# tebartsch/numpy-quant

Measured on AMD Instinct MI355X. Metric: quantized-int8 samples/sec (ViT-tiny, batch 256) + MatMul GOPS vs int8-MFMA peak, higher is better.
Workload: dtype int8; 1 GPU; vit_image_classifier (reference models/vit graph, ViT-Base/16-224), QModel.__call__ (fused plan), int8, batch 256/GPU; model=vit_image_classifier_no_weights.onnx (ViT-Base/16-224), global_batch=256, seq_len=197, parallelism=replicas x1, executor=fused plan, hipGraph replay

## Files before the change

include/nqk.h:

```cpp
#ifndef NQK_H
#define NQK_H

#include <stddef.h>
#include <stdint.h>

#ifdef __cplusplus
extern "C" {
#endif

enum nqk_dtype { NQK_I8 = 1, NQK_I16 = 2, NQK_I32 = 3, NQK_I64 = 4, NQK_F32 = 5 };

enum nqk_zp_flags {
  NQK_ZP_NONE = 0,
  NQK_ZP_SCALAR = 1,
  NQK_ZP_ROW = 2,
  NQK_ZP_COL = 4,
  NQK_ZP_KCONST = 8,
  NQK_ZP_FULL = 16
};

int nqk_init(int device);
int nqk_device_count(int* count);
const char* nqk_last_error(void);
int nqk_malloc(void** ptr, size_t bytes);
// ... 145 lines not shown
  int64_t ln_zp;
} nqk_epilogue;
int nqk_pack_b(const int8_t* bt, int8_t* out, int64_t N, int64_t K, int64_t ldb);
int nqk_pack_b4(const int8_t* bt, uint8_t* out, int64_t N, int64_t K, int64_t ldb);
int nqk_pack_pg(const int8_t* bt, int8_t* out, int64_t N, int64_t K, int64_t ldb, int layout);
int nqk_pack_pg4(const int8_t* bt, uint8_t* out, int64_t N, int64_t K, int64_t ldb, int layout);
int nqk_gelu_lut_build(float s_out, int64_t zp_out, int32_t bit_width, float div, float add1, float mul2, void* lut,
                       float* k_out, int32_t* n_out);
int nqk_gelu_lut_capacity(void);
int nqk_gelu_lut_check(float s_out, int64_t zp_out, int32_t bit_width, float div, float add1, float mul2,
                       const void* lut, const float* k, int32_t n, uint64_t* mismatches);
int nqk_qgemm_fused(int epi, const int8_t* a, const int8_t* bt, int64_t batch, int64_t M, int64_t N, int64_t K,
                    int64_t lda, int64_t ldb, const int64_t* bmap, int64_t a_mat_stride, int64_t b_mat_stride,
                    const nqk_epilogue* params);
int nqk_qgemm_last_kernel(void);
int nqk_ln_quant(const float* x, const float* gamma, const float* beta, int8_t* out, int64_t rows, int64_t cols,
                 float eps, float scale, int64_t zp, int bit_width);
int nqk_softmax_quant(const float* x, int8_t* out, int64_t* rowsum, int64_t rows, int64_t cols, int64_t ldo,
                      float scale, int64_t zp, int bit_width);
int nqk_transpose_pad_i8(const int8_t* src, int8_t* dst, int64_t* rowsum, int64_t nb, int64_t R, int64_t C,
                         int64_t Rp);

typedef struct nqk_attention {
  int32_t heads, tokens, hdim, ld_out, bit_width, pad0;
  int64_t zq, zk;
  float s_qk, div;
  float s_p, s_pv;
  int64_t zp_p, zv;
  float s_ctx, pad1;
  int64_t zp_ctx;
} nqk_attention;
int nqk_attention_fused(const int8_t* q, const int8_t* k, const int8_t* v, int8_t* ctx, int64_t batch_heads,
                        const nqk_attention* params);

int nqk_selftest_fastmath(unsigned long long* counts_dev, uint32_t* examples_dev);
int nqk_selftest_gelu_filter(unsigned long long* stats_dev);

int nqk_comm_unique_id(void* id128);
int nqk_comm_init(const void* id128, int nranks, int rank);
int nqk_comm_bcast(void* buf, size_t bytes, int root);
int nqk_comm_gather(const void* send, void* recv, size_t bytes_per_rank, int root);
int nqk_comm_barrier(void);
int nqk_comm_destroy(void);

#ifdef __cplusplus
}
#endif
// ... 2 lines not shown
```

numpy-quant_amd/csrc/nqk_attn.hip:

```cpp
#include <type_traits>

#include "nqk_common.h"
#include "nqk_numerics.h"

#ifndef NQK_ATTN_DIAG
#define NQK_ATTN_DIAG 0
#endif
#ifndef NQK_ATTN_EXPW
#define NQK_ATTN_EXPW 4
#endif
#ifndef NQK_ATTN_PK
#define NQK_ATTN_PK 1
#endif
#ifndef NQK_ATTN_PQ2
#define NQK_ATTN_PQ2 1
#endif
#ifndef NQK_ATTN_EXP2
#define NQK_ATTN_EXP2 1
#endif
#ifndef NQK_ATTN_PREL
#define NQK_ATTN_PREL 1
#endif
#ifndef NQK_ATTN_PM_R
#define NQK_ATTN_PM_R 0x1.3p-22f
// ... 15 lines not shown
  (void)hipMemcpyFromSymbol(out, HIP_SYMBOL(g_attn_stats), 4 * sizeof(unsigned long long));
  const unsigned long long z[4] = {0, 0, 0, 0};
  if (reset) (void)hipMemcpyToSymbol(HIP_SYMBOL(g_attn_stats), z, sizeof(z));
  return 0;
}
#define NQK_ATTN_COUNT(i) \
  do { if ((threadIdx.x & 63) == 0) atomicAdd(&g_attn_stats[i], 1ull); } while (0)
#else
#define NQK_ATTN_COUNT(i) do { } while (0)
#endif
namespace {

typedef int v4i __attribute__((ext_vector_type(4)));
typedef int v16i __attribute__((ext_vector_type(16)));

struct AttnArgs {
  int T, H, ld_out, EST, PST, n2;
  int zq, zk, zp, zv;
  int kq, kp;
  float s_qk, div, s_p, s_pv, s_ctx;
  double rdiv, rs_p, zp_p, rs_ctx, zp_ctx, lo, hi;
  float inv_div, rs_ctx_f, zp_p_f, zp_ctx_f, lo_f, hi_f;
  float s_qkd;
};

__device__ __forceinline__ int swz64a(int row, int chunk) { return row * 64 + ((chunk ^ ((row >> 2) & 3)) << 4); }

__device__ __forceinline__ int sum16a(v4i c) {
  int s = __builtin_amdgcn_sdot4(c[0], 0x01010101, 0, false);
  s = __builtin_amdgcn_sdot4(c[1], 0x01010101, s, false);
  s = __builtin_amdgcn_sdot4(c[2], 0x01010101, s, false);
  return __builtin_amdgcn_sdot4(c[3], 0x01010101, s, false);
}

__device__ __forceinline__ float div_rc_w(float x, double rc) { return (float)((double)x * rc); }

__device__ __forceinline__ int quant_w(float x, float s, double rs, double zp, double lo, double hi) {
  const float t = div_rc_w(x, rs);
  const double u = zp + (double)t;
  return (int)__builtin_rint(__builtin_fmin(__builtin_fmax(u, lo), hi));
}

__device__ __forceinline__ int xor32i(int x) {
  const auto r = __builtin_amdgcn_permlane32_swap(x, x, false, false);
  return (threadIdx.x & 32) ? (int)r[0] : (int)r[1];
}
// ... 145 lines not shown
#pragma unroll
          for (int jj = 0; jj < 4; ++jj) qs[jj] = (int)o[jj];
        } else if constexpr (FAST) {
          v2f_t dd0, dd1;
          const v2f_t t0 = v2f_t{o[0], o[1]} * v2f_t{a.rs_ctx_f, a.rs_ctx_f};
          const v2f_t t1 = v2f_t{o[2], o[3]} * v2f_t{a.rs_ctx_f, a.rs_ctx_f};
          const v2f_t s0 = round_magic2(t0, a.lo_f - a.zp_ctx_f, a.hi_f - a.zp_ctx_f, 0x1.8p23f + a.zp_ctx_f, dd0);
          const v2f_t s1 = round_magic2(t1, a.lo_f - a.zp_ctx_f, a.hi_f - a.zp_ctx_f, 0x1.8p23f + a.zp_ctx_f, dd1);
          const float m0 = __builtin_fmaf(__builtin_fabsf(t0[0]), 0x1p-21f, __builtin_fabsf(dd0[0]));
          const float m1 = __builtin_fmaf(__builtin_fabsf(t0[1]), 0x1p-21f, __builtin_fabsf(dd0[1]));
          const float m2 = __builtin_fmaf(__builtin_fabsf(t1[0]), 0x1p-21f, __builtin_fabsf(dd1[0]));
          const float m3 = __builtin_fmaf(__builtin_fabsf(t1[1]), 0x1p-21f, __builtin_fabsf(dd1[1]));
          const uint32_t wm = __builtin_elementwise_max(__builtin_elementwise_max(__float_as_uint(m0), __float_as_uint(m1)),
                                                        __builtin_elementwise_max(__float_as_uint(m2), __float_as_uint(m3)));
          packed = pack4_low(s0, s1);
          if (__builtin_expect(__any(wm >= __float_as_uint(0x1.fffffcp-2f)), 0)) {
            NQK_ATTN_COUNT(3);
#pragma unroll
            for (int jj = 0; jj < 4; ++jj) {
              const int qv = quant_w(o[jj], a.s_ctx, a.rs_ctx, a.zp_ctx, a.lo, a.hi);
              packed = (packed & ~(0xffu << (8 * jj))) | ((uint32_t)(qv & 0xff) << (8 * jj));
            }
          }
          if (m < T) *reinterpret_cast<uint32_t*>(orow + d0) = packed;
          __builtin_amdgcn_sched_barrier(0);
          continue;
        } else {
#pragma unroll
          for (int jj = 0; jj < 4; ++jj) qs[jj] = quant_w(o[jj], a.s_ctx, a.rs_ctx, a.zp_ctx, a.lo, a.hi);
        }
#pragma unroll
        for (int jj = 0; jj < 4; ++jj) packed |= ((uint32_t)(qs[jj] & 0xff)) << (8 * jj);
        if (m < T) *reinterpret_cast<uint32_t*>(orow + d0) = packed;
        __builtin_amdgcn_sched_barrier(0);
      }
  };
  for (int rt = wave; rt < (TAILR ? NT - 1 : NT); rt += 4) {
    const int m0 = rt * 32, m = m0 + r32;
    v4i qb[2];
    const int nrowterm = q_rows(m, qb);
    int rp;
    v16i acc2[2];
    float e[NT][16];
    float mx = -__builtin_inff();
    float mn = __builtin_inff();
    int imx = INT32_MIN, imn = INT32_MAX;
#pragma unroll
    for (int c = 0; c < NT; ++c) {
      v16i acc;
#pragma unroll
      for (int qq = 0; qq < 4; ++qq) {
        if (pad_group(c, qq)) {
#pragma unroll
          for (int j = 0; j < 4; ++j) acc[4 * qq + j] = 0;
          continue;
        }
        const v4i ck = *reinterpret_cast<const v4i*>(colK + c * 32 + 8 * qq + 4 * h);
#pragma unroll
        for (int j = 0; j < 4; ++j) acc[4 * qq + j] = nrowterm - ck[j];
      }
// ... 341 lines not shown
          rp += qv;
          packed |= ((uint32_t)(qv & 0xff)) << (8 * j);
        }
        dw[qq] = (int)packed;
        __builtin_amdgcn_sched_barrier(0);
      }
      }
      const int xa = xor32i(h ? dw[0] : dw[2]);
      const int xb = xor32i(h ? dw[1] : dw[3]);
      v4i pb;
      if (h) { pb[0] = xa; pb[1] = dw[2]; pb[2] = xb; pb[3] = dw[3]; }
      else   { pb[0] = dw[0]; pb[1] = xa; pb[2] = dw[1]; pb[3] = xb; }
#pragma unroll
      for (int j = 0; j < 2; ++j) {
        const v4i va = *reinterpret_cast<const v4i*>(Vt + vt_row(j * 32 + r32) + (2 * c + h) * 16);
        if constexpr ((NQK_ATTN_DIAG & 32) != 0) acc2[j][c] ^= va[0] ^ pb[j];
        else acc2[j] = __builtin_amdgcn_mfma_i32_32x32x32_i8(va, pb, acc2[j], 0, 0, 0);
      }
    }
    rp += xor32i(rp);
    ctx_store(m, rp, acc2);
  }
  if constexpr (TAILR) {
    if (wave == (NT - 1) % 4) {
      const int rt = NT - 1, m = rt * 32 + r32;
      v4i qb[2];
      const int nrowterm = q_rows(m, qb);
      int rp;
      v16i acc2[2];
#pragma unroll
      for (int c = 0; c < NT; ++c) {
        v16i acc;
#pragma unroll
        for (int qq = 0; qq < 4; ++qq) {
          if (pad_group(c, qq)) {
#pragma unroll
            for (int j = 0; j < 4; ++j) acc[4 * qq + j] = 0;
            continue;
          }
          const v4i ck = *reinterpret_cast<const v4i*>(colK + c * 32 + 8 * qq + 4 * h);
#pragma unroll
          for (int j = 0; j < 4; ++j) acc[4 * qq + j] = nrowterm - ck[j];
        }
#pragma unroll
        for (int s = 0; s < 2; ++s) {
          const v4i ka = *reinterpret_cast<const v4i*>(Ks + swz64a(c * 32 + r32, 2 * s + h));
          acc = __builtin_amdgcn_mfma_i32_32x32x32_i8(ka, qb[s], acc, 0, 0, 0);
// ... 218 lines not shown
  if (tid < A16_KP) {
    const int8_t* kr = Ks + tid * 64;
    colK[tid] = (sum16a(*reinterpret_cast<const v4i*>(kr)) + sum16a(*reinterpret_cast<const v4i*>(kr + 16)) +
                 sum16a(*reinterpret_cast<const v4i*>(kr + 32)) + sum16a(*reinterpret_cast<const v4i*>(kr + 48))) * a.zq -
                a.kq;
  }
  if (tid < 256) {
    const int d = tid >> 2, ch = tid & 3;
    const int8_t* vr = Vt + (ch * 64 + d) * 64;
    int s = sum16a(*reinterpret_cast<const v4i*>(vr)) + sum16a(*reinterpret_cast<const v4i*>(vr + 16)) +
            sum16a(*reinterpret_cast<const v4i*>(vr + 32)) + sum16a(*reinterpret_cast<const v4i*>(vr + 48));
    s += __shfl_xor(s, 1, 64);
    s += __shfl_xor(s, 2, 64);
    if (ch == 0) colV[d] = s * a.zp - a.kp;
  }
  __syncthreads();

  const int fo = l15 * 64 + 16 * (g ^ a16_sw(l15));
  const float pqlo = a.lo_f - a.zp_p_f, pqhi = a.hi_f - a.zp_p_f, pmagic = 0x1.8p23f + a.zp_p_f;
  auto q_frag = [&](int rt) __attribute__((always_inline)) {
    const int mq = rt * 16 + l15;
    return *reinterpret_cast<const v4i*>(q + (mq < T ? mq : T - 1) * 64 + g * 16);
  };
  v4i qnext = q_frag(wave);
  for (int rt = wave; rt < NT; rt += NW) {
    const int m = rt * 16 + l15;
    const v4i qb = NQK_ATTN16_QPF ? qnext : q_frag(rt);
    int nrowterm;
    {
      int rq = sum16a(qb);
      rq += xor16i(rq);
      rq += xor32i(rq);
      nrowterm = -(rq * a.zk);
      asm volatile("" : "+v"(nrowterm));
    }
    float e[NT][4];
    int imx = INT32_MIN, imn = INT32_MAX;
    float mx = -__builtin_inff();
#pragma unroll
    for (int c = 0; c < NT; ++c) {
      const v4i ck = *reinterpret_cast<const v4i*>(colK + 16 * c + 4 * g);
      v4i acc = v4i{nrowterm - ck[0], nrowterm - ck[1], nrowterm - ck[2], nrowterm - ck[3]};
      const v4i ka = *reinterpret_cast<const v4i*>(Ks + c * 1024 + fo);
      acc = __builtin_amdgcn_mfma_i32_16x16x64_i8(ka, qb, acc, 0, 0, 0);
#pragma unroll
      for (int r = 0; r < 4; r += 2) {
        v2f_t y = v2f_t{(float)acc[r], (float)acc[r + 1]} * v2f_t{a.s_qkd, a.s_qkd};
        if (c == NT - 1) {
          const int n0 = 192 + 8 * (r >> 1) + 2 * g;
          y = y + v2f_t{n0 < T ? 0.0f : -__builtin_inff(), n0 + 1 < T ? 0.0f : -__builtin_inff()};
          mx = __builtin_fmaxf(mx, __builtin_fmaxf(y[0], y[1]));
        } else {
          imx = max(imx, max(acc[r], acc[r + 1]));
          imn = min(imn, min(acc[r], acc[r + 1]));
        }
        e[c][r] = y[0];
        e[c][r + 1] = y[1];
      }
    }
    if (NQK_ATTN16_QPF && rt + NW < NT) qnext = q_frag(rt + NW);
    mx = __builtin_fmaxf(mx, (float)imx * a.s_qkd);
    mx = __builtin_fmaxf(mx, xor16f(mx));
    mx = __builtin_fmaxf(mx, xor32f(mx));
    const float nm = -mx;
    const float mn = (float)imn * a.s_qkd;
    const bool esafe = __all(mn + nm >= NP_EXP_SAFE_LO);
#pragma unroll
    for (int c = 0; c < NT; ++c) {
#pragma unroll
      for (int r = 0; r < 4; r += 2) {
        const v2f_t xa = v2f_t{e[c][r], e[c][r + 1]} + v2f_t{nm, nm};
        const v2f_t x = (c < NT - 1 && esafe) ? np_expf_safe2(xa) : np_expf_nonpos2(xa);
        e[c][r] = x[0];
        e[c][r + 1] = x[1];
      }
      __builtin_amdgcn_sched_barrier(0);
    }
    float tot;
    {
      v2f_t a0 = v2f_t{e[0][0], e[0][1]}, a1 = v2f_t{e[6][0], e[6][1]};
      a0 = a0 + v2f_t{e[0][2], e[0][3]};
      a1 = a1 + v2f_t{e[6][2], e[6][3]};
#pragma unroll
// ... 103 lines not shown
      const v4i cv = *reinterpret_cast<const v4i*>(colV + d0);
      float o[4];
#pragma unroll
      for (int jj = 0; jj < 4; ++jj) o[jj] = (float)(acc2[mm][jj] - rowp - cv[jj]) * a.s_pv;
      v2f_t dd0, dd1;
      const v2f_t t0 = v2f_t{o[0], o[1]} * v2f_t{a.rs_ctx_f, a.rs_ctx_f};
      const v2f_t t1 = v2f_t{o[2], o[3]} * v2f_t{a.rs_ctx_f, a.rs_ctx_f};
      const v2f_t s0 = round_magic2(t0, a.lo_f - a.zp_ctx_f, a.hi_f - a.zp_ctx_f, 0x1.8p23f + a.zp_ctx_f, dd0);
      const v2f_t s1 = round_magic2(t1, a.lo_f - a.zp_ctx_f, a.hi_f - a.zp_ctx_f, 0x1.8p23f + a.zp_ctx_f, dd1);
      const float m0 = __builtin_fmaf(__builtin_fabsf(t0[0]), 0x1p-21f, __builtin_fabsf(dd0[0]));
      const float m1 = __builtin_fmaf(__builtin_fabsf(t0[1]), 0x1p-21f, __builtin_fabsf(dd0[1]));
      const float m2 = __builtin_fmaf(__builtin_fabsf(t1[0]), 0x1p-21f, __builtin_fabsf(dd1[0]));
      const float m3 = __builtin_fmaf(__builtin_fabsf(t1[1]), 0x1p-21f, __builtin_fabsf(dd1[1]));
      const uint32_t wm = __builtin_elementwise_max(__builtin_elementwise_max(__float_as_uint(m0), __float_as_uint(m1)),
                                                    __builtin_elementwise_max(__float_as_uint(m2), __float_as_uint(m3)));
      uint32_t packed = pack4_low(s0, s1);
      if (__builtin_expect(__any(wm >= __float_as_uint(0x1.fffffcp-2f)), 0)) {
#pragma unroll
        for (int jj = 0; jj < 4; ++jj) {
          const int qv = quant_w(o[jj], a.s_ctx, a.rs_ctx, a.zp_ctx, a.lo, a.hi);
          packed = (packed & ~(0xffu << (8 * jj))) | ((uint32_t)(qv & 0xff) << (8 * jj));
        }
      }
      if (m < T) *reinterpret_cast<uint32_t*>(orow + d0) = packed;
    }
  }
}
}
}

using namespace nqk;

extern "C" int nqk_attention_fused(const int8_t* q, const int8_t* k, const int8_t* v, int8_t* ctx,
                                   int64_t batch_heads, const nqk_attention* p) {
  if (batch_heads <= 0) return 0;
  const int T = p->tokens;
  if (p->hdim != 64) return fail("nqk_attention_fused: head dimension 64 expected");
  if (T < 1 || T > 224) return fail("nqk_attention_fused: 1 <= tokens <= 224 expected");
  if (p->heads < 1 || batch_heads % p->heads) return fail("nqk_attention_fused: batch_heads % heads != 0");
  if (p->ld_out < p->heads * 64) return fail("nqk_attention_fused: ld_out < heads * 64");
  if (p->bit_width < 2 || p->bit_width > 8) return fail("nqk_attention_fused: 2 <= bit_width <= 8 expected");
  auto small = [](int64_t z, int64_t lim) { return z >= -lim && z <= lim; };
  if (!small(p->zq, 4096) || !small(p->zk, 4096) || !small(p->zp_p, 1024) || !small(p->zv, 1024))
    return fail("nqk_attention_fused: zero points beyond the int32-exact range");
  if ((((uintptr_t)q) | ((uintptr_t)k) | ((uintptr_t)v)) & 15) return fail("nqk_attention_fused: unaligned Q/K/V");
  if ((((uintptr_t)ctx) & 3) || (p->ld_out & 3)) return fail("nqk_attention_fused: ctx / ld_out not 4-byte aligned");
  auto normal = [](float x) { return __builtin_fabsf(x) >= 0x1p-100f && __builtin_fabsf(x) <= 0x1p100f; };
  if (!normal(p->s_p) || !normal(p->s_ctx) || !normal(p->div))
    return fail("nqk_attention_fused: scales / divisor outside [2^-100, 2^100]");
  if (batch_heads > 0x7fffffff) return fail("nqk_attention_fused: too many (image, head) pairs");
  const int NT = (T + 31) / 32;
  AttnArgs a{};
  a.T = T;
  a.H = p->heads;
  a.ld_out = p->ld_out;
  int est = (T + 3) / 4 * 4;
  if (((est / 4) & 1) == 0) est += 4;
  a.EST = est;
  a.PST = NT * 32 + 16;
  a.n2 = 0;
  if (T > 128) {
    a.n2 = T / 2;
    a.n2 -= a.n2 % 8;
  }
  a.zq = (int)p->zq;
  a.zk = (int)p->zk;
  a.zp = (int)p->zp_p;
  a.zv = (int)p->zv;
  a.kq = a.zq * a.zk * 64;
  a.kp = a.zp * a.zv * T;
  a.s_qk = p->s_qk;
  a.div = p->div;
  a.rdiv = 1.0 / (double)p->div;
  a.s_p = p->s_p;
  a.rs_p = 1.0 / (double)p->s_p;
  a.zp_p = (double)p->zp_p;
// ... 50 lines not shown
```

numpy-quant_amd/numpy_quant/_lib.py:

```python
from __future__ import annotations

import ctypes
import os

_HERE = os.path.dirname(os.path.abspath(__file__))
LIB_PATH = os.path.join(_HERE, "libnqk.so")

NQK_I8, NQK_I16, NQK_I32, NQK_I64, NQK_F32 = 1, 2, 3, 4, 5
ZP_NONE, ZP_SCALAR, ZP_ROW, ZP_COL, ZP_KCONST, ZP_FULL = 0, 1, 2, 4, 8, 16
ADD, SUB, MUL, DIV = 0, 1, 2, 3
NEG, EXP, ERF, SQRT, RELU, SIGMOID, RECIP, TANH = range(8)
IMG_NHWC, IMG_NCHW = 0, 1

_p = ctypes.c_void_p
_i = ctypes.c_int
_l = ctypes.c_int64
_f = ctypes.c_float
_lp = ctypes.POINTER(ctypes.c_int64)

class Epilogue(ctypes.Structure):
    _fields_ = [("zp_flags", ctypes.c_int32), ("bit_width", ctypes.c_int32), ("group_cols", ctypes.c_int32),
                ("tokens", ctypes.c_int32), ("heads", ctypes.c_int32), ("hdim", ctypes.c_int32),
                ("ld_out", ctypes.c_int32), ("col_absmax", ctypes.c_int32),
                ("zpa", ctypes.c_int64), ("zpb", ctypes.c_int64), ("kdim", ctypes.c_int64),
                ("row", ctypes.c_void_p), ("col", ctypes.c_void_p),
                ("s_acc", ctypes.c_float * 3), ("s_out", ctypes.c_float * 3), ("zp_out", ctypes.c_int64 * 3),
                ("out", ctypes.c_void_p * 3), ("bias", ctypes.c_void_p), ("resid", ctypes.c_void_p),
                ("div", ctypes.c_float), ("add1", ctypes.c_float), ("mul2", ctypes.c_float),
                ("b_packed", ctypes.c_int32), ("colterm", ctypes.c_void_p), ("bt_pg", ctypes.c_void_p),
                ("gelu_lut", ctypes.c_void_p), ("lut_k", ctypes.c_float * 5), ("lut_n", ctypes.c_int32),
                ("col_l1max", ctypes.c_int32),
                ("ln_gamma", ctypes.c_void_p), ("ln_beta", ctypes.c_void_p), ("ln_out", ctypes.c_void_p),
                ("ln_eps", ctypes.c_float), ("ln_scale", ctypes.c_float), ("ln_zp", ctypes.c_int64)]


class Attention(ctypes.Structure):
    _fields_ = [("heads", ctypes.c_int32), ("tokens", ctypes.c_int32), ("hdim", ctypes.c_int32),
                ("ld_out", ctypes.c_int32), ("bit_width", ctypes.c_int32), ("pad0", ctypes.c_int32),
                ("zq", ctypes.c_int64), ("zk", ctypes.c_int64),
                ("s_qk", ctypes.c_float), ("div", ctypes.c_float), ("s_p", ctypes.c_float), ("s_pv", ctypes.c_float),
                ("zp_p", ctypes.c_int64), ("zv", ctypes.c_int64),
                ("s_ctx", ctypes.c_float), ("pad1", ctypes.c_float), ("zp_ctx", ctypes.c_int64)]


SIGNATURES = {
    "nqk_init": [_i],
    "nqk_device_count": [ctypes.POINTER(_i)],
    "nqk_malloc": [ctypes.POINTER(_p), ctypes.c_size_t],
    "nqk_free": [_p],
    "nqk_memcpy_h2d": [_p, _p, ctypes.c_size_t],
    "nqk_memcpy_d2h": [_p, _p, ctypes.c_size_t],
    "nqk_memcpy_d2d": [_p, _p, ctypes.c_size_t],
    "nqk_memset": [_p, _i, ctypes.c_size_t],
    "nqk_sync": [],
    "nqk_stream": [ctypes.POINTER(_p)],
    "nqk_set_stream": [_i],
    "nqk_stream_fork": [],
    "nqk_stream_join": [],
    "nqk_timer_start": [],
    "nqk_timer_stop": [],
    "nqk_timer_ms": [ctypes.POINTER(_f)],
# ... 135 lines not shown
```

numpy-quant_amd/numpy_quant/graph.py:

```python
from __future__ import annotations

import ctypes
from typing import List, Sequence, Union

import numpy as np

from . import _lib
from .device import POOL, DeviceArray, sync
from .tensor import FTensor


class DeviceGraph:

    def __init__(self, qmodel, example_inputs: Sequence[Union[np.ndarray, FTensor]], topk=None):
        _lib.ensure_init()
        from . import kernels as KM
        if KM.TIMER is not None:
            raise RuntimeError("DeviceGraph: kernels.TIMER is active; its events would be frozen into the graph")
        self.q = qmodel
        self.topk = topk
        self.staging: List[FTensor] = []
        for a in example_inputs:
            if isinstance(a, FTensor):
                self.staging.append(FTensor(a.dev.copy()))
            elif isinstance(a, np.ndarray) and a.dtype == np.float32:
                self.staging.append(FTensor(np.ascontiguousarray(a)))
            else:
                raise ValueError("DeviceGraph: float32 inputs only (int64 inputs are host tensors)")
        self.plan = None
        if qmodel._plan is not None or (qmodel.fuse and not qmodel.keep_values):
            from .plan import compile_plan
            self.plan = compile_plan(qmodel)
        self.exec = ctypes.c_void_p()
        self.outs: list = []
        self.blocks = []
        saved = qmodel._plan
        qmodel._plan = self.plan
        try:
            self._forward()
            sync()
            self.deq_cache = dict(qmodel._deq_cache)
            POOL.capture = []
            _lib.call("nqk_graph_begin")
            try:
                outs = self._forward()
            except BaseException:
                _lib.call("nqk_graph_abort")
                raise
            _lib.call("nqk_graph_end", ctypes.byref(self.exec))
            self.outs = outs
        finally:
            if POOL.capture is not None:
                self.blocks, POOL.capture = POOL.capture, None
            qmodel._plan = saved

# ... 46 lines not shown
```

numpy-quant_amd/numpy_quant/plan.py:

```python
from __future__ import annotations

import ctypes
import os
import math
from typing import Optional

import numpy as np

from . import _lib
from . import kernels as KM
from .device import DeviceArray
from .tensor import FTensor, QTensor

EPI_QKV, EPI_SCORES, EPI_PV, EPI_RESID, EPI_GELU = 0, 1, 2, 3, 4

_EPI_NAMES = {EPI_QKV: "qkv", EPI_SCORES: "scores", EPI_PV: "pv", EPI_RESID: "resid", EPI_GELU: "gelu"}

FUSED_ATTENTION = True
FUSED_EMBED = True
LN_GATHER = True
SPLIT_STREAMS = True


Epilogue = _lib.Epilogue
# ... 453 lines not shown
                                             4 * (n * hw * self.kk + self.kk * self.kout + n * (hw + 1) * self.kout)),
                         unit="flop32")
        m.add.outputs[0].data = FTensor(out)
        m.conv_out.data = FusedAway(m.conv_out.name)


class LnGather:

    def __init__(self, qmodel, ln):
        if ln.op != "LayerNormalization":
            raise NoMatch("LayerNormalization expected")
        out = ln.outputs[0]
        g = _only(out.outputs, "LN consumer")
        if g.op != "Gather" or g.inputs[0] is not out:
            raise NoMatch("Gather consumer expected")
        idx = g.inputs[1]
        if not (idx.inputs and idx.inputs[0].op == "Constant"):
            raise NoMatch("constant Gather indices expected")
        ax = int(ln.attrs.get("axis", -1))
        gax = int(g.attrs.get("axis", 0))
        if ax != -1 or gax in (-1,):
            raise NoMatch("LN over the last axis, Gather over another one")
        self.ln, self.g, self.nodes = ln, g, {ln, g}

    def run(self, qmodel, times=None, profile=False):
        from .model import onnx_operator_implementation
        x = self.ln.inputs[0].data
        if not isinstance(x, FTensor) or int(self.g.attrs.get("axis", 0)) % x.dev.ndim == x.dev.ndim - 1:
            raise ValueError("LN/Gather pushdown needs a float input gathered off the last axis")
        xs = x.take(self.g.inputs[1].data, axis=int(self.g.attrs.get("axis", 0)))
        args = [xs] + [qmodel._dequant_input(v) if isinstance(v.data, QTensor) else v.data for v in self.ln.inputs[1:]]
        self.g.outputs[0].data = onnx_operator_implementation("LayerNormalization", args, self.ln.attrs)[0]
        self.ln.outputs[0].data = FusedAway(self.ln.outputs[0].name)


class FusedLayer:
    def __init__(self, qmodel, m: LayerMatch):
        self.m = m
        self.bw = qmodel.bit_width
        qp = qmodel.quant_params
        deq = qmodel._dequant_input
        cf = lambda v: _const_float(qmodel, v)
        self.g1, self.be1 = cf(m.ln1.inputs[1]).dev, cf(m.ln1.inputs[2]).dev
        self.g2, self.be2 = cf(m.ln2.inputs[1]).dev, cf(m.ln2.inputs[2]).dev
        self.eps1 = _f32(m.ln1.attrs.get("epsilon", 1e-5))
        self.eps2 = _f32(m.ln2.attrs.get("epsilon", 1e-5))
        self.p_ln1, self.p_ln2 = qp[m.ln1_out.name], qp[m.ln2_out.name]
        self.p_sm, self.p_ctx, self.p_h = qp[m.sm_out.name], qp[m.rs3_out.name], qp[m.h_out.name]
        self.p_head = {r: qp[m.roles[r]["tr_out"].name] for r in "qkv"}
        bts, cols, biases, self.s_w = [], [], [], {}
        for r in "qkv":
            w = m.roles[r]["w"].data
            bt, col = w.weight_operand()
            bts.append(bt)
            cols.append(col)
            biases.append(deq(m.roles[r]["bias"]).dev)
# ... 10 lines not shown
        self.s_wo, self.s_w1, self.s_w2 = m.wo.data.scale, m.w1.data.scale, m.w2.data.scale
        self.bias_o, self.bias_1, self.bias_2 = deq(m.bo).dev, deq(m.b1).dev, deq(m.b2).dev
        self.F = self.bt_1.shape[0]
        self.bp = {k: _pack_b(b, self.bw) for k, b in (("qkv", self.bt_qkv), ("o", self.bt_o), ("1", self.bt_1),
                                                        ("2", self.bt_2))}
        self.bpg = {k: _pack_pg(b, self.bw, lay, nibbles=self.bp[k] is not None and self.bp[k][1] == 2)
                    for k, b, lay in (("qkv", self.bt_qkv, 0), ("o", self.bt_o, 1), ("1", self.bt_1, 0),
                                      ("2", self.bt_2, 1))}
        self.cmax = {k: _absmax(c) for k, c in (("qkv", self.col_qkv), ("o", self.col_o), ("1", self.col_1),
                                                 ("2", self.col_2))}
        self.l1max = {k: _l1max(b) for k, b in (("qkv", self.bt_qkv), ("o", self.bt_o), ("1", self.bt_1),
                                                 ("2", self.bt_2))}
        self.ct = {k: _colterm(c, _zp(p)) for k, c, p in (("qkv", self.col_qkv, self.p_ln1), ("o", self.col_o, self.p_ctx),
                                                          ("1", self.col_1, self.p_ln2), ("2", self.col_2, self.p_h))}
        if self.D != m.heads * m.hdim or self.bt_o.shape != (self.D, self.D) or self.bt_2.shape != (self.D, self.F):
            raise NoMatch("layer dimensions")
        self.glut = _gelu_lut(self.p_h, self.bw, m.gelu_div, m.gelu_add, m.gelu_mul)
        zs = [_zp(self.p_head["q"]), _zp(self.p_head["k"]), _zp(self.p_sm), _zp(self.p_head["v"])]
        self.attn_fused = (FUSED_ATTENTION and m.hdim == 64 and 1 <= m.tokens <= 224 and
                           abs(zs[0]) <= 4096 and abs(zs[1]) <= 4096 and abs(zs[2]) <= 1024 and abs(zs[3]) <= 1024)
        self.ln_fuse = self.D == 192 and not os.environ.get("NQK_NO_LNFUSE")
        self.next_ln = None
        self.ln1_by_prev = False

    def _epi(self, **kw) -> Epilogue:
        e = Epilogue()
        e.bit_width = self.bw
        e.group_cols = kw.pop("group_cols", 1 << 30)
        e.tokens, e.heads, e.hdim = self.m.tokens, self.m.heads, self.m.hdim
        e.div, e.add1, e.mul2 = kw.pop("div", 1.0), kw.pop("add1", 0.0), kw.pop("mul2", 1.0)
        for k, v in kw.items():
            if k in ("s_acc", "s_out", "zp_out", "out"):
                arr = getattr(e, k)
                for i, x in enumerate(v):
                    arr[i] = x
            else:
                setattr(e, k, v)
        return e

    @staticmethod
    def _ln_into(e, g, b, eps, p, out):
        e.ln_gamma, e.ln_beta, e.ln_out = g.ptr, b.ptr, out.ptr
        e.ln_eps, e.ln_scale, e.ln_zp = eps, _f32(p.scale), _zp(p)

    def _b(self, e, key, bt):
        bp = self.bp[key]
# ... 10 lines not shown
                      s_acc=[_f32(np.float32(pq.scale) * np.float32(pk.scale))], out=[w["s"].ptr], div=m.div)
        _gemm(EPI_SCORES, w["q"], w["k"], B * H, T, T, Dh, Dh, Dh, None, T * Dh, T * Dh, e)
        call("nqk_softmax_quant", w["s"].vp, w["p"].vp, None, B * H * T, T, Tp,
             _f32(self.p_sm.scale), _zp(self.p_sm), bw)
        e = self._epi(zp_flags=_lib.ZP_ROW | _lib.ZP_COL | _lib.ZP_KCONST, zpa=_zp(self.p_sm), zpb=_zp(pv_), kdim=T,
                      s_acc=[_f32(np.float32(self.p_sm.scale) * np.float32(pv_.scale))],
                      s_out=[_f32(self.p_ctx.scale)], zp_out=[_zp(self.p_ctx)], out=[w["ctx"].ptr], ld_out=D)
        _gemm(EPI_PV, w["p"], w["vt"], B * H, T, Dh, Tp, Tp, Tp, None, T * Tp, Dh * Tp, e)

    def run(self, ws: "Workspace", streams: Streams = _ONE_STREAM):
        m = self.m
        x = m.x_in.data
        if isinstance(x, QTensor):
            streams.join()
            x = x.dequantize()
        if not isinstance(x, FTensor):
            raise ValueError("fused layer input must be a float or quantized tensor")
        B, T, D = x.dev.shape
        if T != m.tokens or D != self.D:
            raise ValueError(f"layer input {x.dev.shape} does not match the graph ({m.tokens}, {self.D})")
        H, Dh, F = m.heads, m.hdim, self.F
        Tp = (T + 15) // 16 * 16
        w = ws.get(B, T, Tp, H, Dh, D, F, unfused_attention=not self.attn_fused)
        x2 = DeviceArray((B, T, D), np.float32)
        if not self.attn_fused:
            streams.join()
            streams = _ONE_STREAM
        streams.halves(B, lambda s_idx, i0, nb: self._run_part(w, x.dev, w["x1"], x2, i0, nb, s_idx, streams.parts))
        m.x_out.data = FTensor(x2)

    def _run_part(self, w, xd, x1d, x2d, i0, nb, s_idx=0, parts=1):
        m, bw = self.m, self.bw
        lag = _stream_lag() if parts > 1 else None
        if lag and s_idx > 0:
            _lib.call("nqk_event_wait", _lag_event(s_idx - 1))

        def mark(point):
            if lag == point and s_idx + 1 < parts:
                _lib.call("nqk_event_record", _lag_event(s_idx))
        T, D = m.tokens, self.D
        H, Dh, F = m.heads, m.hdim, self.F
        Mrows = nb * T
        Tp = (T + 15) // 16 * 16
        r0 = i0 * T

        def rows(arr, ncol):
            return arr.offset_view(r0 * ncol, (Mrows, ncol))

        x, x1, x2 = (rows(t.reshape((t.size // D, D)), D) for t in (xd, x1d, x2d))
        lnq, ln2q, ctx, hh = rows(w["lnq"], D), rows(w["ln2q"], D), rows(w["ctx"], D), rows(w["h"], F)
        hq = i0 * H * T * Dh
        q, k, v = (w[r].offset_view(hq, (nb * H * T, Dh)) for r in "qkv")
        call = _lib.call
        if not self.ln1_by_prev:
            _ln_quant(x, self.g1, self.be1, lnq, Mrows, D, self.eps1, self.p_ln1, bw)
        mark("ln1")
        s_a = np.float32(self.p_ln1.scale)
        e = self._epi(zp_flags=_lib.ZP_COL, zpa=_zp(self.p_ln1), group_cols=D, col=self.col_qkv.ptr,
                      col_absmax=self.cmax["qkv"], col_l1max=self.l1max["qkv"], colterm=_ptr(self.ct["qkv"]),
                      s_acc=[_f32(s_a * np.float32(self.s_w[r])) for r in "qkv"],
                      s_out=[_f32(self.p_head[r].scale) for r in "qkv"],
                      zp_out=[_zp(self.p_head[r]) for r in "qkv"],
                      out=[q.ptr, k.ptr, v.ptr], bias=self.bias_qkv.ptr)
        _gemm(EPI_QKV, lnq, self._b(e, "qkv", self.bt_qkv), 1, Mrows, 3 * D, D, D, D, None, 0, 0, e)
        mark("qkv")
        pq, pk, pv_ = self.p_head["q"], self.p_head["k"], self.p_head["v"]
        if self.attn_fused:
            a = _lib.Attention()
            a.heads, a.tokens, a.hdim, a.ld_out, a.bit_width = H, T, Dh, D, bw
            a.zq, a.zk = _zp(pq), _zp(pk)
            a.s_qk, a.div = _f32(np.float32(pq.scale) * np.float32(pk.scale)), m.div
            a.s_p, a.zp_p = _f32(self.p_sm.scale), _zp(self.p_sm)
            a.s_pv, a.zv = _f32(np.float32(self.p_sm.scale) * np.float32(pv_.scale)), _zp(pv_)
            a.s_ctx, a.zp_ctx = _f32(self.p_ctx.scale), _zp(self.p_ctx)
            t0 = KM.TIMER.begin() if KM.TIMER is not None else None
            call("nqk_attention_fused", q.vp, k.vp, v.vp, ctx.vp, nb * H, ctypes.byref(a))
            if t0 is not None:
                KM.TIMER.end("attention", t0, (2 * 2 * nb * H * T * T * Dh, 3 * nb * H * T * Dh + nb * T * D))
        else:
            self._attention_unfused(w, nb, T, Tp, H, Dh, D)
        mark("attn")
        e = self._epi(zp_flags=_lib.ZP_COL, zpa=_zp(self.p_ctx), col=self.col_o.ptr, col_absmax=self.cmax["o"], col_l1max=self.l1max["o"],
                      colterm=_ptr(self.ct["o"]),
                      s_acc=[_f32(np.float32(self.p_ctx.scale) * np.float32(self.s_wo))], bias=self.bias_o.ptr,
                      resid=x.ptr, out=[x1.ptr])
        if self.ln_fuse:
            self._ln_into(e, self.g2, self.be2, self.eps2, self.p_ln2, ln2q)
        _gemm(EPI_RESID, ctx, self._b(e, "o", self.bt_o), 1, Mrows, D, D, D, D, None, 0, 0, e)
        if not self.ln_fuse:
            _ln_quant(x1, self.g2, self.be2, ln2q, Mrows, D, self.eps2, self.p_ln2, bw)
        e = self._epi(zp_flags=_lib.ZP_COL, zpa=_zp(self.p_ln2), col=self.col_1.ptr, col_absmax=self.cmax["1"], col_l1max=self.l1max["1"],
                      colterm=_ptr(self.ct["1"]),
                      s_acc=[_f32(np.float32(self.p_ln2.scale) * np.float32(self.s_w1))], bias=self.bias_1.ptr,
                      s_out=[_f32(self.p_h.scale)], zp_out=[_zp(self.p_h)], out=[hh.ptr],
                      div=m.gelu_div, add1=m.gelu_add, mul2=m.gelu_mul)
        if self.glut is not None:
            e.gelu_lut, e.lut_n = self.glut[0].ptr, self.glut[2]
            for j, kv in enumerate(self.glut[1]):
                e.lut_k[j] = kv
        _gemm(EPI_GELU, ln2q, self._b(e, "1", self.bt_1), 1, Mrows, F, D, D, D, None, 0, 0, e)
        e = self._epi(zp_flags=_lib.ZP_COL, zpa=_zp(self.p_h), col=self.col_2.ptr, col_absmax=self.cmax["2"], col_l1max=self.l1max["2"],
                      colterm=_ptr(self.ct["2"]),
                      s_acc=[_f32(np.float32(self.p_h.scale) * np.float32(self.s_w2))], bias=self.bias_2.ptr,
                      resid=x1.ptr, out=[x2.ptr])
        nl = self.next_ln
        if nl is not None:
            self._ln_into(e, nl.g1, nl.be1, nl.eps1, nl.p_ln1, lnq)
        _gemm(EPI_RESID, hh, self._b(e, "2", self.bt_2), 1, Mrows, D, F, F, F, None, 0, 0, e)


def _pack_b(bt, bit_width=8):
    N, K = bt.shape
# ... 80 lines not shown
        raise ValueError("fused GEMM operands must be 16-byte padded")
    need_a = (batch - 1) * a_ms + (M - 1) * lda + K if batch > 1 else (M - 1) * lda + K
    need_b = (batch - 1) * b_ms + (N - 1) * ldb + K if batch > 1 else (N - 1) * ldb + K
    if e.b_packed:
        need_b = ((N + 255) // 256 * 256) * K // (2 if e.b_packed == 2 else 1)
    if need_a > a.size or need_b > bt.size * bt.dtype.itemsize:
        raise ValueError("fused GEMM operand smaller than its shape")
    t0 = KM.TIMER.begin() if KM.TIMER is not None else None
    _lib.call("nqk_qgemm_fused", epi, a.vp, bt.vp, batch, M, N, K, lda, ldb,
              _lib.i64arr(bmap) if bmap is not None else None, a_ms, b_ms, ctypes.byref(e))
    if t0 is not None:
        name = _EPI_NAMES[epi]
        out_b = 8 * M * N if epi == EPI_RESID else (M * N if epi in (EPI_QKV, EPI_GELU) else 0)
        if epi == EPI_RESID:
            name = "down" if K > N else "out"
        KM.TIMER.end("qgemm_" + name, t0, (2 * batch * M * N * K, batch * (M * K + N * K + out_b)))


class Workspace:

    def __init__(self):
        self.key = None
        self.bufs = {}

    def get(self, B, T, Tp, H, Dh, D, F, unfused_attention=True):
        key = (B, T, Tp, H, Dh, D, F)
        if key != self.key:
            M = B * T
            self.bufs = {
                "lnq": DeviceArray((M, D), np.int8), "ln2q": DeviceArray((M, D), np.int8),
                "q": DeviceArray((B * H * T, Dh), np.int8), "k": DeviceArray((B * H * T, Dh), np.int8),
                "v": DeviceArray((B * H * T, Dh), np.int8),
                "ctx": DeviceArray((M, D), np.int8), "h": DeviceArray((M, F), np.int8),
                "x1": DeviceArray((B, T, D), np.float32),
            }
            self.key = key
        if unfused_attention and "s" not in self.bufs:
            self.bufs.update({"vt": DeviceArray((B * H, Dh, Tp), np.int8),
                              "s": DeviceArray((B * H, T, T), np.float32),
                              "p": DeviceArray((B * H, T, Tp), np.int8)})
        return self.bufs


class FusedAwayError(RuntimeError):
    """Reading a FusedAway value."""


class FusedAway:

    def __init__(self, name):
        self.name = name

    def _error(self):
        return FusedAwayError(f"value {self.name!r} was computed inside a fused plan step and not kept; "
                              "set QModel.keep_values = True to read intermediates")

    def __getattr__(self, attr):
        if attr.startswith("__") and attr.endswith("__"):
            raise AttributeError(attr)
        raise self._error()

    def __array__(self, *args, **kwargs):
        raise self._error()

# ... 46 lines not shown
                    claimed[n] = layer
        placed = set()
        for node in qmodel.nodes:
            layer = claimed.get(node)
            if layer is None:
                self.steps.append(("node", node))
            elif isinstance(layer, LnGather):
                if node is layer.g:
                    self.steps.append(("ln_gather", layer))
            elif isinstance(layer, FusedEmbed):
                if node is layer.m.conv:
                    self.steps.append(("embed_pre", layer))
                elif node is layer.m.add:
                    self.steps.append(("embed", layer))
            elif id(layer) not in placed:
                placed.add(id(layer))
                self.steps.append(("layer", layer))
                self.fused += 1
        for (k0, a), (k1, b) in zip(self.steps, self.steps[1:]):
            if (k0 == "layer" and k1 == "layer" and a.ln_fuse and b.ln_fuse and b.m.x_in is a.m.x_out and
                    (a.D, a.F, a.m.heads, a.m.hdim, a.m.tokens, a.attn_fused) ==
                    (b.D, b.F, b.m.heads, b.m.hdim, b.m.tokens, b.attn_fused)):
                a.next_ln, b.ln1_by_prev = b, True
        self.internal = [v for node in qmodel.nodes if node in claimed for v in node.outputs]

    def run(self, qmodel, times=None, profile=False):
        streams = Streams(self.split, int(os.environ.get("NQK_STREAMS", "2")))
        for v in self.internal:
            v.data = FusedAway(v.name)
        try:
            for kind, obj in self.steps:
                if kind == "node":
                    streams.join()
                    qmodel._run_node(obj, times, profile)
                elif kind == "embed_pre":
                    obj.pre(qmodel)
                elif kind == "embed":
                    obj.run(qmodel, streams)
                elif kind == "ln_gather":
                    streams.join()
                    obj.run(qmodel, times, profile)
                else:
                    obj.run(self.ws, streams)
        finally:
            _lib.call("nqk_set_stream", 0)
            streams.join()


def compile_plan(qmodel) -> Plan:
    return Plan(qmodel)
```

Baseline: 29570 samples/s.

## Compute only CLS token rows in final transformer layer before LN/Gather

When the last layer's output only feeds a LayerNorm+Gather of token 0, the final layer now runs attention for just the first query row (new q_rows parameter in the fused attention kernel) and runs the out-projection/MLP on B rows instead of B*T. The full output becomes a lazily computed deferred tensor, or is fused away inside the graph executor. This removes the attention queries, out-proj and MLP work for the remaining tokens in the last layer. In exchange it adds CLS-specific workspace buffers, strided copies, and a plan rewrite that depends on the graph gathering index 0.

```diff
diff --git a/include/nqk.h b/include/nqk.h
--- a/include/nqk.h
+++ b/include/nqk.h
@@ -191,7 +191,7 @@
                          int64_t Rp);
 
 typedef struct nqk_attention {
-  int32_t heads, tokens, hdim, ld_out, bit_width, pad0;
+  int32_t heads, tokens, hdim, ld_out, bit_width, q_rows;
   int64_t zq, zk;
   float s_qk, div;
   float s_p, s_pv;
diff --git a/numpy-quant_amd/csrc/nqk_attn.hip b/numpy-quant_amd/csrc/nqk_attn.hip
--- a/numpy-quant_amd/csrc/nqk_attn.hip
+++ b/numpy-quant_amd/csrc/nqk_attn.hip
@@ -61,6 +61,7 @@
   double rdiv, rs_p, zp_p, rs_ctx, zp_ctx, lo, hi;
   float inv_div, rs_ctx_f, zp_p_f, zp_ctx_f, lo_f, hi_f;
   float s_qkd;
+  int QR;
 };
 
 __device__ __forceinline__ int swz64a(int row, int chunk) { return row * 64 + ((chunk ^ ((row >> 2) & 3)) << 4); }
@@ -252,7 +253,7 @@
               packed = (packed & ~(0xffu << (8 * jj))) | ((uint32_t)(qv & 0xff) << (8 * jj));
             }
           }
-          if (m < T) *reinterpret_cast<uint32_t*>(orow + d0) = packed;
+          if (m < a.QR) *reinterpret_cast<uint32_t*>(orow + d0) = packed;
           __builtin_amdgcn_sched_barrier(0);
           continue;
         } else {
@@ -261,11 +262,12 @@
         }
 #pragma unroll
         for (int jj = 0; jj < 4; ++jj) packed |= ((uint32_t)(qs[jj] & 0xff)) << (8 * jj);
-        if (m < T) *reinterpret_cast<uint32_t*>(orow + d0) = packed;
+        if (m < a.QR) *reinterpret_cast<uint32_t*>(orow + d0) = packed;
         __builtin_amdgcn_sched_barrier(0);
       }
   };
-  for (int rt = wave; rt < (TAILR ? NT - 1 : NT); rt += 4) {
+  const int ntq = (a.QR + 31) >> 5;
+  for (int rt = wave; rt < (TAILR ? min(ntq, NT - 1) : ntq); rt += 4) {
     const int m0 = rt * 32, m = m0 + r32;
     v4i qb[2];
     const int nrowterm = q_rows(m, qb);
@@ -653,7 +655,7 @@
     ctx_store(m, rp, acc2);
   }
   if constexpr (TAILR) {
-    if (wave == (NT - 1) % 4) {
+    if (wave == (NT - 1) % 4 && ntq == NT) {
       const int rt = NT - 1, m = rt * 32 + r32;
       v4i qb[2];
       const int nrowterm = q_rows(m, qb);
@@ -918,8 +920,9 @@
     const int mq = rt * 16 + l15;
     return *reinterpret_cast<const v4i*>(q + (mq < T ? mq : T - 1) * 64 + g * 16);
   };
+  const int ntq = (a.QR + 15) >> 4;
   v4i qnext = q_frag(wave);
-  for (int rt = wave; rt < NT; rt += NW) {
+  for (int rt = wave; rt < ntq; rt += NW) {
     const int m = rt * 16 + l15;
     const v4i qb = NQK_ATTN16_QPF ? qnext : q_frag(rt);
     int nrowterm;
@@ -954,7 +957,7 @@
         e[c][r + 1] = y[1];
       }
     }
-    if (NQK_ATTN16_QPF && rt + NW < NT) qnext = q_frag(rt + NW);
+    if (NQK_ATTN16_QPF && rt + NW < ntq) qnext = q_frag(rt + NW);
     mx = __builtin_fmaxf(mx, (float)imx * a.s_qkd);
     mx = __builtin_fmaxf(mx, xor16f(mx));
     mx = __builtin_fmaxf(mx, xor32f(mx));
@@ -1104,7 +1107,7 @@
           packed = (packed & ~(0xffu << (8 * jj))) | ((uint32_t)(qv & 0xff) << (8 * jj));
         }
       }
-      if (m < T) *reinterpret_cast<uint32_t*>(orow + d0) = packed;
+      if (m < a.QR) *reinterpret_cast<uint32_t*>(orow + d0) = packed;
     }
   }
 }
@@ -1119,6 +1122,7 @@
   const int T = p->tokens;
   if (p->hdim != 64) return fail("nqk_attention_fused: head dimension 64 expected");
   if (T < 1 || T > 224) return fail("nqk_attention_fused: 1 <= tokens <= 224 expected");
+  if (p->q_rows < 0 || p->q_rows > T) return fail("nqk_attention_fused: 0 <= q_rows <= tokens expected");
   if (p->heads < 1 || batch_heads % p->heads) return fail("nqk_attention_fused: batch_heads % heads != 0");
   if (p->ld_out < p->heads * 64) return fail("nqk_attention_fused: ld_out < heads * 64");
   if (p->bit_width < 2 || p->bit_width > 8) return fail("nqk_attention_fused: 2 <= bit_width <= 8 expected");
@@ -1134,6 +1138,7 @@
   const int NT = (T + 31) / 32;
   AttnArgs a{};
   a.T = T;
+  a.QR = p->q_rows ? p->q_rows : T;
   a.H = p->heads;
   a.ld_out = p->ld_out;
   int est = (T + 3) / 4 * 4;
diff --git a/numpy-quant_amd/numpy_quant/_lib.py b/numpy-quant_amd/numpy_quant/_lib.py
--- a/numpy-quant_amd/numpy_quant/_lib.py
+++ b/numpy-quant_amd/numpy_quant/_lib.py
@@ -36,7 +36,7 @@
 
 class Attention(ctypes.Structure):
     _fields_ = [("heads", ctypes.c_int32), ("tokens", ctypes.c_int32), ("hdim", ctypes.c_int32),
-                ("ld_out", ctypes.c_int32), ("bit_width", ctypes.c_int32), ("pad0", ctypes.c_int32),
+                ("ld_out", ctypes.c_int32), ("bit_width", ctypes.c_int32), ("q_rows", ctypes.c_int32),
                 ("zq", ctypes.c_int64), ("zk", ctypes.c_int64),
                 ("s_qk", ctypes.c_float), ("div", ctypes.c_float), ("s_p", ctypes.c_float), ("s_pv", ctypes.c_float),
                 ("zp_p", ctypes.c_int64), ("zv", ctypes.c_int64),
diff --git a/numpy-quant_amd/numpy_quant/graph.py b/numpy-quant_amd/numpy_quant/graph.py
--- a/numpy-quant_amd/numpy_quant/graph.py
+++ b/numpy-quant_amd/numpy_quant/graph.py
@@ -31,6 +31,9 @@
         if qmodel._plan is not None or (qmodel.fuse and not qmodel.keep_values):
             from .plan import compile_plan
             self.plan = compile_plan(qmodel)
+            for kind, step in self.plan.steps:
+                if kind == "layer":
+                    step.keep_deferred = False
         self.exec = ctypes.c_void_p()
         self.outs: list = []
         self.blocks = []
diff --git a/numpy-quant_amd/numpy_quant/plan.py b/numpy-quant_amd/numpy_quant/plan.py
--- a/numpy-quant_amd/numpy_quant/plan.py
+++ b/numpy-quant_amd/numpy_quant/plan.py
@@ -499,16 +499,54 @@
         if ax != -1 or gax in (-1,):
             raise NoMatch("LN over the last axis, Gather over another one")
         self.ln, self.g, self.nodes = ln, g, {ln, g}
+        self.cls_layer = None
+
+    def gathers_token0(self) -> bool:
+        idx = np.asarray(_const_node_value(self.g.inputs[1])[0])
+        return int(self.g.attrs.get("axis", 0)) == 1 and idx.size == 1 and int(idx.reshape(-1)[0]) == 0
 
     def run(self, qmodel, times=None, profile=False):
         from .model import onnx_operator_implementation
+        if self.cls_layer is not None:
+            c = self.cls_layer.cls_out.dev
+            idx = np.asarray(self.g.inputs[1].data.data)
+            xs = FTensor(c.reshape((c.shape[0],) + idx.shape + (c.shape[2],)))
+        else:
+            xs = self._gather()
+        args = [xs] + [qmodel._dequant_input(v) if isinstance(v.data, QTensor) else v.data for v in self.ln.inputs[1:]]
+        self.g.outputs[0].data = onnx_operator_implementation("LayerNormalization", args, self.ln.attrs)[0]
+        self.ln.outputs[0].data = FusedAway(self.ln.outputs[0].name)
+
+    def _gather(self):
         x = self.ln.inputs[0].data
         if not isinstance(x, FTensor) or int(self.g.attrs.get("axis", 0)) % x.dev.ndim == x.dev.ndim - 1:
             raise ValueError("LN/Gather pushdown needs a float input gathered off the last axis")
-        xs = x.take(self.g.inputs[1].data, axis=int(self.g.attrs.get("axis", 0)))
-        args = [xs] + [qmodel._dequant_input(v) if isinstance(v.data, QTensor) else v.data for v in self.ln.inputs[1:]]
-        self.g.outputs[0].data = onnx_operator_implementation("LayerNormalization", args, self.ln.attrs)[0]
-        self.ln.outputs[0].data = FusedAway(self.ln.outputs[0].name)
+        return x.take(self.g.inputs[1].data, axis=int(self.g.attrs.get("axis", 0)))
+
+
+class DeferredRows(FTensor):
+
+    def __init__(self, name, shape, thunk):
+        self.name, self._shape, self._thunk = name, tuple(shape), thunk
+        self._dev = self._host = None
+
+    @property
+    def dev(self):
+        if self._dev is None:
+            if self._thunk is None:
+                raise FusedAwayError(f"value {self.name!r}: only its token-0 rows were computed, and a later run "
+                                     "has reused the layer's workspace; read it before the next run, or set "
+                                     "QModel.keep_values = True")
+            self._dev, self._thunk = self._thunk(), None
+        return self._dev
+
+    @property
+    def shape(self):
+        from .tensor import ITensor
+        return ITensor(np.array(self._shape, dtype=np.int64))
+
+    def expire(self):
+        self._thunk = None
 
 
 class FusedLayer:
@@ -565,6 +603,10 @@
         self.ln_fuse = self.D == 192 and not os.environ.get("NQK_NO_LNFUSE")
         self.next_ln = None
         self.ln1_by_prev = False
+        self.cls_tail = False
+        self.keep_deferred = True
+        self.cls_out = None
+        self.deferred = None
 
     def _epi(self, **kw) -> Epilogue:
         e = Epilogue()
@@ -621,6 +663,9 @@
         H, Dh, F = m.heads, m.hdim, self.F
         Tp = (T + 15) // 16 * 16
         w = ws.get(B, T, Tp, H, Dh, D, F, unfused_attention=not self.attn_fused)
+        if self.cls_tail:
+            self._run_cls(ws, w, x, B, streams)
+            return
         x2 = DeviceArray((B, T, D), np.float32)
         if not self.attn_fused:
             streams.join()
@@ -628,7 +673,39 @@
         streams.halves(B, lambda s_idx, i0, nb: self._run_part(w, x.dev, w["x1"], x2, i0, nb, s_idx, streams.parts))
         m.x_out.data = FTensor(x2)
 
-    def _run_part(self, w, xd, x1d, x2d, i0, nb, s_idx=0, parts=1):
+    def _run_cls(self, ws, w, x, B, streams):
+        from .device import copy_strided
+        m = self.m
+        T, D = m.tokens, self.D
+        c = ws.cls(B, D, self.F)
+        out = DeviceArray((B, 1, D), np.float32)
+
+        def part(s_idx, i0, nb):
+            def rows(arr):
+                ncol = arr.shape[-1]
+                return arr.offset_view(i0 * ncol, (nb, ncol))
+            self._run_part(w, x.dev, None, None, i0, nb, s_idx, streams.parts, q_rows=1)
+            copy_strided(w["ctx"], c["ctx"], (nb, D), (T * D, 1), (D, 1), i0 * T * D, i0 * D)
+            copy_strided(x.dev, c["x"], (nb, D), (T * D, 1), (D, 1), i0 * T * D, i0 * D)
+            self._back(rows(c["x"]), rows(c["ctx"]), rows(c["x1"]), rows(c["ln2q"]), rows(c["h"]),
+                       rows(out.reshape((B, D))), None, nb, ln_fuse=False)
+
+        streams.halves(B, part)
+        self.cls_out = FTensor(out)
+        if self.keep_deferred:
+            self.deferred = DeferredRows(m.x_out.name, (B, T, D), lambda: self._all_rows(w, x, B))
+            m.x_out.data = self.deferred
+        else:
+            m.x_out.data = FusedAway(m.x_out.name)
+
+    def _all_rows(self, w, x, B):
+        _lib.call("nqk_set_stream", 0)
+        _lib.call("nqk_stream_join")
+        x2 = DeviceArray((B, self.m.tokens, self.D), np.float32)
+        self._run_part(w, x.dev, w["x1"], x2, 0, B, front=False)
+        return x2
+
+    def _run_part(self, w, xd, x1d, x2d, i0, nb, s_idx=0, parts=1, q_rows=0, front=True):
         m, bw = self.m, self.bw
         lag = _stream_lag() if parts > 1 else None
         if lag and s_idx > 0:
@@ -646,27 +723,28 @@
         def rows(arr, ncol):
             return arr.offset_view(r0 * ncol, (Mrows, ncol))
 
-        x, x1, x2 = (rows(t.reshape((t.size // D, D)), D) for t in (xd, x1d, x2d))
+        x = rows(xd.reshape((xd.size // D, D)), D)
         lnq, ln2q, ctx, hh = rows(w["lnq"], D), rows(w["ln2q"], D), rows(w["ctx"], D), rows(w["h"], F)
         hq = i0 * H * T * Dh
         q, k, v = (w[r].offset_view(hq, (nb * H * T, Dh)) for r in "qkv")
         call = _lib.call
-        if not self.ln1_by_prev:
-            _ln_quant(x, self.g1, self.be1, lnq, Mrows, D, self.eps1, self.p_ln1, bw)
-        mark("ln1")
-        s_a = np.float32(self.p_ln1.scale)
-        e = self._epi(zp_flags=_lib.ZP_COL, zpa=_zp(self.p_ln1), group_cols=D, col=self.col_qkv.ptr,
-                      col_absmax=self.cmax["qkv"], col_l1max=self.l1max["qkv"], colterm=_ptr(self.ct["qkv"]),
-                      s_acc=[_f32(s_a * np.float32(self.s_w[r])) for r in "qkv"],
-                      s_out=[_f32(self.p_head[r].scale) for r in "qkv"],
-                      zp_out=[_zp(self.p_head[r]) for r in "qkv"],
-                      out=[q.ptr, k.ptr, v.ptr], bias=self.bias_qkv.ptr)
-        _gemm(EPI_QKV, lnq, self._b(e, "qkv", self.bt_qkv), 1, Mrows, 3 * D, D, D, D, None, 0, 0, e)
-        mark("qkv")
+        if front:
+            if not self.ln1_by_prev:
+                _ln_quant(x, self.g1, self.be1, lnq, Mrows, D, self.eps1, self.p_ln1, bw)
+            mark("ln1")
+            s_a = np.float32(self.p_ln1.scale)
+            e = self._epi(zp_flags=_lib.ZP_COL, zpa=_zp(self.p_ln1), group_cols=D, col=self.col_qkv.ptr,
+                          col_absmax=self.cmax["qkv"], col_l1max=self.l1max["qkv"], colterm=_ptr(self.ct["qkv"]),
+                          s_acc=[_f32(s_a * np.float32(self.s_w[r])) for r in "qkv"],
+                          s_out=[_f32(self.p_head[r].scale) for r in "qkv"],
+                          zp_out=[_zp(self.p_head[r]) for r in "qkv"],
+                          out=[q.ptr, k.ptr, v.ptr], bias=self.bias_qkv.ptr)
+            _gemm(EPI_QKV, lnq, self._b(e, "qkv", self.bt_qkv), 1, Mrows, 3 * D, D, D, D, None, 0, 0, e)
+            mark("qkv")
         pq, pk, pv_ = self.p_head["q"], self.p_head["k"], self.p_head["v"]
         if self.attn_fused:
             a = _lib.Attention()
-            a.heads, a.tokens, a.hdim, a.ld_out, a.bit_width = H, T, Dh, D, bw
+            a.heads, a.tokens, a.hdim, a.ld_out, a.bit_width, a.q_rows = H, T, Dh, D, bw, q_rows
             a.zq, a.zk = _zp(pq), _zp(pk)
             a.s_qk, a.div = _f32(np.float32(pq.scale) * np.float32(pk.scale)), m.div
             a.s_p, a.zp_p = _f32(self.p_sm.scale), _zp(self.p_sm)
@@ -675,18 +753,27 @@
             t0 = KM.TIMER.begin() if KM.TIMER is not None else None
             call("nqk_attention_fused", q.vp, k.vp, v.vp, ctx.vp, nb * H, ctypes.byref(a))
             if t0 is not None:
-                KM.TIMER.end("attention", t0, (2 * 2 * nb * H * T * T * Dh, 3 * nb * H * T * Dh + nb * T * D))
+                qr = q_rows or T
+                KM.TIMER.end("attention", t0, (2 * 2 * nb * H * qr * T * Dh, nb * H * Dh * (qr + 2 * T) + nb * qr * D))
         else:
             self._attention_unfused(w, nb, T, Tp, H, Dh, D)
         mark("attn")
+        if q_rows:
+            return
+        x1, x2 = (rows(t.reshape((t.size // D, D)), D) for t in (x1d, x2d))
+        self._back(x, ctx, x1, ln2q, hh, x2, lnq, Mrows, self.ln_fuse)
+
+    def _back(self, x, ctx, x1, ln2q, hh, x2, lnq, Mrows, ln_fuse):
+        m, bw = self.m, self.bw
+        D, F = self.D, self.F
         e = self._epi(zp_flags=_lib.ZP_COL, zpa=_zp(self.p_ctx), col=self.col_o.ptr, col_absmax=self.cmax["o"], col_l1max=self.l1max["o"],
                       colterm=_ptr(self.ct["o"]),
                       s_acc=[_f32(np.float32(self.p_ctx.scale) * np.float32(self.s_wo))], bias=self.bias_o.ptr,
                       resid=x.ptr, out=[x1.ptr])
-        if self.ln_fuse:
+        if ln_fuse:
             self._ln_into(e, self.g2, self.be2, self.eps2, self.p_ln2, ln2q)
         _gemm(EPI_RESID, ctx, self._b(e, "o", self.bt_o), 1, Mrows, D, D, D, D, None, 0, 0, e)
-        if not self.ln_fuse:
+        if not ln_fuse:
             _ln_quant(x1, self.g2, self.be2, ln2q, Mrows, D, self.eps2, self.p_ln2, bw)
         e = self._epi(zp_flags=_lib.ZP_COL, zpa=_zp(self.p_ln2), col=self.col_1.ptr, col_absmax=self.cmax["1"], col_l1max=self.l1max["1"],
                       colterm=_ptr(self.ct["1"]),
@@ -813,6 +900,8 @@
     def __init__(self):
         self.key = None
         self.bufs = {}
+        self.cls_key = None
+        self.cls_bufs = {}
 
     def get(self, B, T, Tp, H, Dh, D, F, unfused_attention=True):
         key = (B, T, Tp, H, Dh, D, F)
@@ -831,6 +920,14 @@
                               "s": DeviceArray((B * H, T, T), np.float32),
                               "p": DeviceArray((B * H, T, Tp), np.int8)})
         return self.bufs
+
+    def cls(self, B, D, F):
+        if self.cls_key != (B, D, F):
+            self.cls_bufs = {"x": DeviceArray((B, D), np.float32), "ctx": DeviceArray((B, D), np.int8),
+                             "x1": DeviceArray((B, D), np.float32), "ln2q": DeviceArray((B, D), np.int8),
+                             "h": DeviceArray((B, F), np.int8)}
+            self.cls_key = (B, D, F)
+        return self.cls_bufs
 
 
 class FusedAwayError(RuntimeError):
@@ -923,12 +1020,25 @@
                     (a.D, a.F, a.m.heads, a.m.hdim, a.m.tokens, a.attn_fused) ==
                     (b.D, b.F, b.m.heads, b.m.hdim, b.m.tokens, b.attn_fused)):
                 a.next_ln, b.ln1_by_prev = b, True
+        self.cls_tails = 0
+        if not os.environ.get("NQK_NO_CLS_TAIL"):
+            layers = {id(l.m.x_out): l for k, l in self.steps if k == "layer"}
+            for k, lg in self.steps:
+                layer = layers.get(id(lg.ln.inputs[0])) if k == "ln_gather" else None
+                if (layer is not None and layer.attn_fused and len(layer.m.x_out.outputs) == 1 and
+                        not any(layer.m.x_out is o for o in qmodel.outputs) and lg.gathers_token0()):
+                    layer.cls_tail, lg.cls_layer = True, layer
+                    self.cls_tails += 1
         self.internal = [v for node in qmodel.nodes if node in claimed for v in node.outputs]
 
     def run(self, qmodel, times=None, profile=False):
         streams = Streams(self.split, int(os.environ.get("NQK_STREAMS", "2")))
         for v in self.internal:
             v.data = FusedAway(v.name)
+        for kind, obj in self.steps:
+            if kind == "layer" and obj.deferred is not None:
+                obj.deferred.expire()
+                obj.deferred = None
         try:
             for kind, obj in self.steps:
                 if kind == "node":
```

New measurement: 31030 samples/s (median of 6 runs). +4.9%, better.
